# kazuto1011/dusty-gan-v2

Hardware: AMD Instinct MI355X
Metric: range-images/sec (G+D step) on dusty_v2 64x512 (higher is better)
Workload: dtype bf16; 1 GPU; configs[2]: configs/gans/dusty_v2.yaml full G+D train step (G step + D step + lazy R1 + ADA + EMA + Adam), 64x512 synthetic; global_batch=64, per_gpu_batch=64, parallelism=dp1, hip_graph=True, d_epilogue_dtype=fp32, pe_table_precomputed=True

## Files before the change

dusty-gan-v2_amd/csrc/api.hip:

```cpp
#include "common.h"

extern "C" int dgv2_abi_version(void) { return 49; }
```

dusty-gan-v2_amd/dgv2_native/__init__.py:

```python
import ctypes
import os

import torch

_HERE = os.path.dirname(os.path.abspath(__file__))
LIB_PATH = os.environ.get("DGV2_LIB_PATH") or os.path.join(os.path.dirname(_HERE), "lib", "libdgv2.so")

F32, BF16 = 0, 1
ABI_VERSION = 49

_c_int, _c_i64, _c_f32, _c_ptr = ctypes.c_int, ctypes.c_int64, ctypes.c_float, ctypes.c_void_p

SIGNATURES = {
    "dgv2_abi_version": [],
    "dgv2_fused_bias_act": [_c_ptr] * 4 + [_c_i64] * 3 + [_c_int, _c_int, _c_f32, _c_f32, _c_int, _c_ptr],
    "dgv2_bias_grad": [_c_ptr, _c_ptr, _c_i64, _c_i64, _c_i64, _c_int, _c_ptr],
    "dgv2_bias_act_bwd": [_c_ptr] * 4 + [_c_i64, _c_int, _c_f32, _c_f32, _c_ptr, _c_i64, _c_int, _c_ptr],
    "dgv2_bias_act_bwd_rs": [_c_ptr] * 4 + [_c_i64, _c_int, _c_f32, _c_f32, _c_ptr, _c_ptr, _c_i64, _c_int, _c_ptr],
    "dgv2_surface_normal": [_c_ptr, _c_ptr] + [_c_int] * 5 + [_c_ptr],
    "dgv2_mbstd_cat_fwd": [_c_ptr] * 3 + [_c_int] * 7 + [_c_ptr],
    "dgv2_mbstd_cat_bwd": [_c_ptr] * 3 + [_c_int] * 7 + [_c_ptr],
    "dgv2_gemm_x3": [_c_ptr, _c_ptr, _c_i64, _c_ptr, _c_ptr, _c_int, _c_int, _c_i64, _c_int, _c_int, _c_i64, _c_i64, _c_i64,
                     _c_int, _c_f32, _c_ptr],
    "dgv2_pe_wgrad_scratch": [_c_ptr] + [_c_int] * 4,
    "dgv2_pe_wgrad": [_c_ptr, _c_ptr, _c_i64, _c_ptr, _c_ptr] + [_c_int] * 4 + [_c_i64, _c_int, _c_ptr],
    "dgv2_mbstd_cat_fwd_x": [_c_ptr] * 3 + [_c_int] * 8 + [_c_ptr],
    "dgv2_mbstd_cat_bwd_x": [_c_ptr] * 3 + [_c_int] * 8 + [_c_ptr],
    "dgv2_scale_cast": [_c_ptr] * 3 + [_c_i64, _c_int, _c_int, _c_int, _c_ptr],
    "dgv2_upfirdn2d": [_c_ptr] * 3 + [_c_int] * 15 + [_c_ptr],
    "dgv2_resample": [_c_ptr] * 4 + [_c_int] * 19 + [_c_ptr],
    "dgv2_resample_tab": [_c_ptr] * 5 + [_c_int] + [_c_ptr] * 3 + [_c_int] * 10 + [_c_ptr],
    "dgv2_resample_tab_add": [_c_ptr] * 6 + [_c_int] + [_c_ptr] * 3 + [_c_int] * 8 + [_c_ptr],
    "dgv2_resample_tab_add_affine": [_c_ptr] * 8 + [_c_int] + [_c_ptr] * 3 + [_c_int] * 8 + [_c_ptr],
    "dgv2_fourier_feature": [_c_ptr] * 5 + [_c_int] * 8 + [_c_ptr],
    "dgv2_downsample_angle": [_c_ptr] * 4 + [_c_int] * 5 + [_c_ptr],
    "dgv2_bmm_nn": [_c_ptr] * 3 + [_c_int] * 6 + [_c_i64, _c_ptr, _c_int, _c_f32, _c_f32, _c_int, _c_int, _c_ptr],
    "dgv2_bmm_tn": [_c_ptr] * 3 + [_c_int] * 7 + [_c_ptr],
    "dgv2_bmm_nn_cat": [_c_ptr] * 4 + [_c_int] * 5 + [_c_ptr, _c_int, _c_f32, _c_f32, _c_int, _c_int, _c_ptr],
    "dgv2_bmm_nn_cat_sq": [_c_ptr] * 4 + [_c_int] * 5 + [_c_ptr, _c_ptr, _c_int, _c_f32, _c_f32, _c_int, _c_int, _c_ptr, _c_int, _c_ptr,
                           _c_ptr],
    "dgv2_bmm_nn_sq": [_c_ptr] * 3 + [_c_int] * 6 + [_c_i64, _c_ptr, _c_ptr, _c_int, _c_f32, _c_f32, _c_ptr, _c_int, _c_int, _c_ptr, _c_int,
                       _c_ptr, _c_ptr],
    "dgv2_modconv_pe_fwd": [_c_ptr] * 4 + [_c_int] * 5 + [_c_ptr, _c_int, _c_f32, _c_f32, _c_int, _c_ptr],
    "dgv2_modconv_pe_fwd_sq": [_c_ptr] * 4 + [_c_int] * 5 + [_c_ptr, _c_ptr, _c_int, _c_f32, _c_f32, _c_int, _c_ptr, _c_int, _c_ptr,
                               _c_ptr],
    "dgv2_modconv_pe_fwd_head": [_c_ptr] * 4 + [_c_int] * 5 + [_c_ptr, _c_ptr, _c_int, _c_f32, _c_f32, _c_int, _c_ptr, _c_int, _c_ptr,
                                 _c_ptr, _c_ptr, _c_ptr],
    "dgv2_kitti_rows": [_c_ptr, _c_ptr, _c_ptr, _c_int, _c_int, _c_ptr],
    "dgv2_kitti_project": [_c_ptr] * 4 + [_c_int] * 4 + [_c_f32, _c_f32, _c_int, _c_ptr],
    "dgv2_fps_scratch": [_c_ptr, _c_int, _c_int],
    "dgv2_fps": [_c_ptr] * 3 + [_c_int] * 3 + [_c_ptr],
    "dgv2_gather_points": [_c_ptr] * 3 + [_c_int] * 4 + [_c_ptr],
    "dgv2_gather_points_grad": [_c_ptr] * 3 + [_c_int] * 4 + [_c_ptr],
    "dgv2_chamfer_fwd": [_c_ptr] * 6 + [_c_int] * 3 + [_c_ptr],
    "dgv2_nn_search": [_c_ptr] * 4 + [_c_int] * 4 + [_c_ptr],
    "dgv2_chamfer_bwd": [_c_ptr] * 8 + [_c_int] * 3 + [_c_ptr],
    "dgv2_emd_approxmatch": [_c_ptr] * 4 + [_c_int] * 3 + [_c_ptr],
    "dgv2_emd_matchcost": [_c_ptr] * 4 + [_c_int] * 3 + [_c_ptr],
    "dgv2_emd_matchcost_grad": [_c_ptr] * 5 + [_c_int] * 3 + [_c_ptr],
    "dgv2_nsgan_loss": [_c_ptr, _c_ptr, _c_ptr, _c_int, _c_int, _c_f32, _c_ptr, _c_ptr, _c_ptr],
    "dgv2_modconv_pe_dgrad_actbwd": [_c_ptr, _c_ptr, _c_ptr, _c_i64] + [_c_ptr] * 5 + [_c_f32, _c_f32] + [_c_int] * 4 + [_c_ptr],
    "dgv2_colmean_lerp": [_c_ptr, _c_ptr, _c_int, _c_int, _c_i64, _c_f32, _c_ptr],
    "dgv2_d_tail_fwd": [_c_ptr] * 6 + [_c_int, _c_int] + [_c_f32] * 4 + [_c_ptr],
    "dgv2_d_tail_bwd": [_c_ptr] * 7 + [_c_int, _c_int] + [_c_f32] * 4 + [_c_ptr],
    "dgv2_rng_fill": [_c_ptr] * 5 + [_c_int, _c_ptr, _c_ptr],
    "dgv2_modconv_up_fwd": [_c_ptr] * 4 + [_c_int] * 7 + [_c_ptr] * 6 + [_c_int, _c_f32, _c_f32, _c_int, _c_ptr, _c_int, _c_ptr,
                            _c_ptr],
    "dgv2_modconv_up_t_lag": [_c_ptr] * 4 + [_c_f32] + [_c_ptr] * 4 + [_c_int] * 9 + [_c_ptr, _c_int, _c_ptr, _c_ptr],
    "dgv2_fir_same_mfma_q8": [_c_ptr] * 3 + [_c_int] * 4 + [_c_ptr],
    "dgv2_resample_tab_q8": [_c_ptr] * 5 + [_c_int] + [_c_ptr] * 3 + [_c_int] * 7 + [_c_ptr],
    "dgv2_fp8_quant_weights": [_c_ptr] * 6 + [_c_int] + [_c_ptr] * 3,
    "dgv2_fp8_dequant": [_c_ptr, _c_ptr, _c_i64, _c_f32, _c_ptr],
    "dgv2_conv_taps_fp8": [_c_ptr] * 4 + [_c_int] * 14 + [_c_ptr, _c_int, _c_ptr, _c_ptr, _c_int, _c_f32, _c_f32, _c_ptr],
    "dgv2_modconv_up_t": [_c_ptr] * 5 + [_c_f32] + [_c_int] * 9 + [_c_ptr],
    "dgv2_up2_lag_sumsq": [_c_ptr] * 5 + [_c_int] * 5 + [_c_ptr, _c_int, _c_ptr, _c_ptr],
    "dgv2_resample_tab_actbwd": [_c_ptr, _c_ptr, _c_ptr, _c_i64, _c_ptr, _c_ptr, _c_ptr] + [_c_ptr] * 3 + [_c_int] + [_c_ptr] * 3
                                + [_c_int] * 7 + [_c_f32, _c_f32, _c_int, _c_ptr],
    "dgv2_fir_same_mfma_prep": [_c_ptr, _c_i64, _c_ptr] + [_c_ptr] * 3 + [_c_int] + [_c_ptr] * 3 + [_c_int] * 3 + [_c_ptr, _c_ptr],
    "dgv2_fir_same_mfma": [_c_ptr] * 3 + [_c_int] * 4 + [_c_ptr],
    "dgv2_fir_same_mfma_actbwd": [_c_ptr, _c_ptr, _c_ptr, _c_i64, _c_ptr, _c_ptr, _c_ptr, _c_ptr] + [_c_int] * 4
                                 + [_c_f32, _c_f32, _c_ptr],
    "dgv2_resample_tab_sq": [_c_ptr] * 5 + [_c_int] + [_c_ptr] * 3 + [_c_int] * 10 + [_c_ptr, _c_int, _c_ptr, _c_ptr],
    "dgv2_bmm_tn_cat": [_c_ptr] * 4 + [_c_int] * 6 + [_c_ptr],
    "dgv2_lerp_list": [_c_ptr] * 3 + [_c_int, _c_f32, _c_ptr],
    "dgv2_adam_prep": [_c_ptr, _c_ptr, _c_f32, _c_f32, _c_ptr],
    "dgv2_adam_step": [_c_ptr] * 5 + [_c_int, _c_ptr] + [_c_f32] * 4 + [_c_ptr],
    "dgv2_pack2d": [_c_ptr] * 4 + [_c_int] * 3 + [_c_ptr],
    "dgv2_unpack2d": [_c_ptr] * 4 + [_c_int] * 3 + [_c_ptr],
    "dgv2_ema_scalar": [_c_ptr] * 3 + [_c_int] + [_c_f32] * 3 + [_c_int, _c_ptr, _c_int, _c_ptr],
    "dgv2_ema_scalar_group": [_c_ptr, _c_ptr, _c_int, _c_ptr, _c_int] + [_c_f32] * 3 + [_c_int, _c_ptr, _c_ptr],
    "dgv2_bmm_nn_small": [_c_ptr] * 4 + [_c_int] * 5 + [_c_ptr],
    "dgv2_bmm_nn_small_act": [_c_ptr] * 4 + [_c_int] * 4 + [_c_ptr, _c_ptr, _c_f32, _c_f32, _c_ptr, _c_ptr, _c_i64, _c_ptr, _c_int,
                              _c_ptr],
    "dgv2_bmm_tn_small": [_c_ptr] * 3 + [_c_int] * 5 + [_c_ptr],
    "dgv2_head_bwd": [_c_ptr] * 5 + [_c_i64] + [_c_ptr] * 7 + [_c_f32, _c_f32] + [_c_int] * 5 + [_c_ptr],
    "dgv2_transpose_list": [_c_ptr] * 5 + [_c_int] * 3 + [_c_ptr],
    "dgv2_mod_prep_all_fwd": [_c_ptr] * 13 + [_c_ptr, _c_int, _c_int, _c_ptr],
    "dgv2_mod_prep_all_bwd": [_c_ptr, _c_i64] + [_c_ptr] * 15 + [_c_ptr, _c_int, _c_int, _c_ptr, _c_i64, _c_ptr],
    "dgv2_mod_prep_all_bwd_scratch": [_c_ptr, _c_ptr, _c_ptr, _c_int, _c_int],
    "dgv2_mod_prep_fwd": [_c_ptr] * 8 + [_c_int] * 9 + [_c_ptr],
    "dgv2_mod_prep_bwd": [_c_ptr] * 11 + [_c_int] * 9 + [_c_ptr],
    "dgv2_sum_squares": [_c_ptr, _c_ptr, _c_i64, _c_int, _c_int, _c_int, _c_ptr],
    "dgv2_conv_fwd": [_c_ptr] * 3 + [_c_int] * 10 + [_c_ptr, _c_int, _c_f32, _c_f32, _c_int, _c_ptr],
    "dgv2_conv_taps": [_c_ptr] * 3 + [_c_int] * 17 + [_c_ptr] + [_c_int] * 3 + [_c_ptr, _c_ptr, _c_int, _c_f32, _c_f32, _c_int,
                                                                               _c_ptr],
    "dgv2_conv_taps_ex": [_c_ptr] * 3 + [_c_int] * 14 + [_c_ptr, _c_int, _c_int, _c_ptr, _c_int, _c_ptr] + [_c_int] * 3
    + [_c_ptr, _c_ptr, _c_int, _c_f32, _c_f32, _c_int, _c_ptr],
    "dgv2_conv_taps_ld": [_c_ptr, _c_int, _c_ptr, _c_ptr] + [_c_int] * 14 + [_c_ptr, _c_int, _c_int, _c_ptr, _c_int, _c_ptr] + [_c_int] * 3
    + [_c_ptr, _c_ptr, _c_int, _c_f32, _c_f32, _c_int, _c_ptr],
    "dgv2_conv_wgrad_direct": [_c_ptr] * 3 + [_c_int] * 10 + [_c_ptr],
    "dgv2_bmm_tn_stream_scratch": [_c_ptr] + [_c_int] * 6,
    "dgv2_bmm_tn_stream": [_c_ptr, _c_ptr, _c_i64, _c_ptr, _c_ptr] + [_c_int] * 6 + [_c_ptr],
    "dgv2_bmm_tn_stream_x": [_c_ptr, _c_ptr, _c_i64, _c_ptr, _c_ptr] + [_c_int] * 7 + [_c_ptr],
    "dgv2_bmm_tn_stream_ld": [_c_ptr, _c_i64, _c_ptr, _c_i64, _c_ptr, _c_ptr] + [_c_int] * 7 + [_c_ptr],
    "dgv2_conv_weight_bank": [_c_ptr] * 8 + [_c_int, _c_int, _c_ptr],
    "dgv2_conv_weight_bank_ex": [_c_ptr] * 10 + [_c_int, _c_int, _c_ptr],
    "dgv2_glin_fwd": [_c_ptr] * 6 + [_c_int] * 3 + [_c_f32, _c_f32, _c_int, _c_f32, _c_int, _c_ptr, _c_ptr],
    "dgv2_glin_dinput": [_c_ptr, _c_int, _c_ptr, _c_i64, _c_ptr, _c_ptr, _c_ptr, _c_ptr, _c_int, _c_int, _c_int, _c_f32, _c_f32,
                         _c_int, _c_ptr],
    "dgv2_glin_dweight": [_c_ptr] * 7 + [_c_int] * 3 + [_c_f32, _c_f32, _c_f32, _c_ptr, _c_ptr],
    "dgv2_conv3x3_dgrad8": [_c_ptr] * 3 + [_c_int] * 5 + [_c_ptr, _c_int, _c_ptr],
    "dgv2_conv3x3_s2_dgrad8": [_c_ptr] * 3 + [_c_int] * 6 + [_c_ptr],
    "dgv2_conv3x3_x3_wgrad_scratch": [_c_ptr] + [_c_int] * 6,
    "dgv2_conv3x3_x3_wgrad": [_c_ptr, _c_ptr, _c_i64] + [_c_ptr] * 2 + [_c_int] * 7 + [_c_f32, _c_int, _c_ptr, _c_ptr],
    "dgv2_conv_x3_images": [_c_ptr] * 3 + [_c_int] * 2 + [_c_ptr],
    "dgv2_conv3x3_x3_dgrad": [_c_ptr] * 4 + [_c_int] * 6 + [_c_ptr, _c_ptr],
    "dgv2_conv3x3_x3_fwd": [_c_ptr] * 3 + [_c_int] * 6 + [_c_ptr, _c_ptr, _c_int, _c_f32, _c_f32, _c_ptr, _c_ptr],
    "dgv2_conv3x3_fwd8": [_c_ptr] * 3 + [_c_int] * 6 + [_c_ptr, _c_ptr, _c_int, _c_f32, _c_f32, _c_int, _c_ptr],
    "dgv2_conv_wgrad_stream_scratch": [_c_ptr] + [_c_int] * 9,
    "dgv2_conv_wgrad_stream": [_c_ptr, _c_ptr, _c_i64, _c_ptr, _c_ptr] + [_c_int] * 10 + [_c_ptr],
    "dgv2_conv_wgrad_stream_pl": [_c_ptr, _c_ptr, _c_i64, _c_ptr, _c_ptr] + [_c_int] * 9 + [_c_f32, _c_int, _c_int, _c_ptr],
    "dgv2_conv_dgrad": [_c_ptr] * 4 + [_c_int] * 11 + [_c_ptr],
    "dgv2_conv_wgrad": [_c_ptr] * 3 + [_c_int] * 11 + [_c_ptr],
    "dgv2_stem_fwd": [_c_ptr] * 4 + [_c_int] * 5 + [_c_f32, _c_f32, _c_int, _c_ptr],
    "dgv2_stem_bwd_scratch": [_c_ptr] + [_c_int] * 4,
    "dgv2_stem_bwd": [_c_ptr] * 4 + [_c_i64] + [_c_ptr] * 4 + [_c_int] * 5 + [_c_f32, _c_f32, _c_int, _c_ptr],
    "dgv2_stem_bwd_skip": [_c_ptr] * 4 + [_c_i64] + [_c_ptr] * 8 + [_c_int] + [_c_ptr] * 3 + [_c_int] * 8 + [_c_f32, _c_f32, _c_int,
                                                                                                        _c_ptr],
    "dgv2_gen_tail_fwd": [_c_ptr] * 7 + [_c_int] * 3 + [_c_f32] * 3 + [_c_ptr],
    "dgv2_gen_tail_bwd": [_c_ptr] * 11 + [_c_int] * 3 + [_c_f32] * 3 + [_c_ptr],
    "dgv2_ada_apply": [_c_ptr] * 8 + [_c_int] * 5 + [_c_ptr],
    "dgv2_ada_sample": [_c_ptr] * 7 + [_c_int] * 3 + [_c_ptr],
    "dgv2_ada_build": [_c_ptr] * 8 + [_c_int] * 4 + [_c_ptr],
    "dgv2_ada_sample_img": [_c_ptr] * 7 + [_c_int, _c_ptr],
    "dgv2_ada_fold": [_c_ptr] * 11 + [_c_int] * 6 + [_c_ptr],
    "dgv2_ada_apply_img": [_c_ptr] * 11 + [_c_int] * 5 + [_c_ptr],
    "dgv2_coords_convert": [_c_ptr] * 4 + [_c_int] * 3 + [_c_f32] * 3 + [_c_int, _c_ptr],
    "dgv2_msml_prepare": [_c_ptr] * 6 + [_c_int] * 5 + [_c_ptr],
    "dgv2_msml_fwd": [_c_ptr] * 7 + [_c_int] * 7 + [_c_ptr],
    "dgv2_msml_bwd": [_c_ptr] * 9 + [_c_int] * 7 + [_c_ptr],
    "dgv2_coords_convert_bwd": [_c_ptr] * 5 + [_c_int] * 3 + [_c_f32, _c_f32, _c_int, _c_ptr],
    "dgv2_fourier_feature_bwd": [_c_ptr] * 6 + [_c_int] * 8 + [_c_ptr],
}


def _load():
    if not os.path.exists(LIB_PATH):
        raise ImportError(
            f"{LIB_PATH} not found: build it with `make` (or __graft_entry__.build()). "
            "The MI355X path has no CPU fallback."
        )
    lib = ctypes.CDLL(LIB_PATH)
    for name, argtypes in SIGNATURES.items():
        fn = getattr(lib, name)
        fn.argtypes = argtypes
        fn.restype = ctypes.c_int
    got = lib.dgv2_abi_version()
    if got != ABI_VERSION:
        raise ImportError(f"libdgv2.so ABI version {got}, binding expects {ABI_VERSION}")
    return lib


lib = _load()


def dtype_code(t):
    if t.dtype == torch.float32:
        return F32
    if t.dtype == torch.bfloat16:
        return BF16
    raise RuntimeError(f"dgv2: unsupported dtype {t.dtype} (float32 / bfloat16 only)")


def check(*tensors):
    for t in tensors:
        if t is None:
            continue
        if not t.is_cuda:
            raise RuntimeError("dgv2: tensor must be a CUDA/HIP tensor (no CPU fallback)")
        if not t.is_contiguous():
            raise RuntimeError("dgv2: tensor must be contiguous")


# ... 63 lines not shown
```

dusty-gan-v2_amd/gans/models/ops/native/conv.py:

```python
import contextlib
import os
from typing import NamedTuple, Optional

import torch
from torch.autograd import Function

import dgv2_native as N
from . import act_resample as _act_resample
from .act_resample import *
from .modgemm import *


class ConvGeom:
    def __init__(self, kh, kw, stride, pad, ring):
        self.kh, self.kw, self.stride, self.pad, self.ring = kh, kw, stride, pad, int(bool(ring))

    def out_hw(self, H, W):
        return (H + 2 * self.pad - self.kh) // self.stride + 1, (W + 2 * self.pad - self.kw) // self.stride + 1

    @property
    def ring3x3(self):
        return bool(self.ring) and (self.kh, self.kw, self.pad) == (3, 3, 1)


def _kstep(t):
    return 32 if t.dtype == torch.bfloat16 else 16


def _conv_taps(y, x, w3, Hg, Wg, in_stride, ioff, out_stride, ooff, taps, hzero, accumulate=False,
               bias=None, act=0, alpha=0.2, scale=1.0, resid=None):
    B, Hin, Win, Cin = x.shape
    O, wtaps, _ = w3.shape
    _, Hy, Wy, _ = y.shape
    arr = (_ct.c_int * (3 * len(taps)))(*[v for t in taps for v in t])
    N.call("dgv2_conv_taps", N.ptr(y), N.ptr(x), N.ptr(w3), B, Hin, Win, Cin, Hg, Wg, O, Hy, Wy, in_stride,
           ioff[0], ioff[1], out_stride, ooff[0], ooff[1], len(taps), wtaps, arr, int(hzero), 1, int(accumulate),
           N.ptr(bias), N.ptr(resid), act, alpha, scale, _dt(x), N.stream())


_FUSED_DGRAD = os.environ.get("DGV2_NO_FUSED_DGRAD") is None


_S2D8 = os.environ.get("DGV2_NO_S2D8") is None


def _conv_taps_ex(y, x, w3, Hg, Wg, in_stride, ioff, out_stride, classes, taps4, extras, hzero, resid=None, ch0=None):
    B, Hin, Win, Cin = x.shape
    O, wtaps, _ = w3.shape
    _, Hy, Wy, ldy = y.shape
    carr = (_ct.c_int * (2 * len(classes)))(*[v for c in classes for v in c])
    tarr = (_ct.c_int * (4 * len(taps4)))(*[v for t in taps4 for v in t])
    earr = (_ct.c_int * max(5 * len(extras), 1))(*[v for e in extras for v in e])
    if ch0 is not None:
        es = y.element_size()
        rp = None if resid is None else resid.data_ptr() + ch0 * es
        return N.try_call("dgv2_conv_taps_ld", y.data_ptr() + ch0 * es, ldy, N.ptr(x), N.ptr(w3), B, Hin, Win, Cin, Hg, Wg,
                          O, Hy, Wy, in_stride, ioff[0], ioff[1], out_stride, len(classes), carr, len(taps4), wtaps,
                          tarr, len(extras), earr, int(hzero), 1, 0, None, rp, 0, 0.2, 1.0, _dt(x), N.stream())
    return N.try_call("dgv2_conv_taps_ex", N.ptr(y), N.ptr(x), N.ptr(w3), B, Hin, Win, Cin, Hg, Wg, O, Hy, Wy,
                      in_stride, ioff[0], ioff[1], out_stride, len(classes), carr, len(taps4), wtaps, tarr,
                      len(extras), earr, int(hzero), 1, 0, None, N.ptr(resid), 0, 0.2, 1.0, _dt(x), N.stream())


def _direct_ok(g, cin):
    return bool(g.ring) and g.kh == g.kw and (g.kh, g.pad) in ((3, 1), (1, 0)) and g.stride in (1, 2) and cin


_CONV8_IMG = os.environ.get("DGV2_NO_CONV8_IMG") is None


_CONV_X3 = os.environ.get("DGV2_NO_CONV_X3") is None


_X3_AUTO = [False, {}]


@contextlib.contextmanager
def x3_auto(on=True, live=None):
    old = tuple(_X3_AUTO)
    _X3_AUTO[0] = bool(on) and _CONV_X3
    _X3_AUTO[1] = dict(live or {})
    try:
        yield
    finally:
        _X3_AUTO[0], _X3_AUTO[1] = old


def _x3_auto_images(wv, fwd):
    O, kh, kw, Cp = wv.shape
    if (not _X3_AUTO[0] or wv.dtype != torch.float32 or not wv.is_cuda or (kh, kw) != (3, 3) or O % 64 or Cp % 8 or Cp < 64
            or not wv.is_contiguous()):
        return None
    n = 3 * (O // 64) * ((Cp + 31) // 32) if fwd else 3 * (Cp // 64) * (O // 32)
    img = torch.empty(n * 2304 * 8, device=wv.device, dtype=torch.bfloat16)
    N.check(wv)
    N.call("dgv2_conv_x3_images", N.ptr(img) if fwd else None, None if fwd else N.ptr(img), N.ptr(wv), O, Cp, N.stream())
    return img


def _conv_fwd_raw(x, w, g, bias=None, act=0, alpha=0.2, scale=1.0, resid=None, w8=None, xexact=0):
    B, H, W, C = x.shape
    O = w.shape[0]
    Ho, Wo = g.out_hw(H, W)
    N.check(x, w, bias)
    y = torch.empty((B, Ho, Wo, O), device=x.device, dtype=x.dtype)
    if (w8 is not None and _CONV8_IMG and x.dtype == torch.bfloat16 and g.ring3x3 and g.stride in (1, 2)
            and N.try_call("dgv2_conv3x3_fwd8", N.ptr(y), N.ptr(x), N.ptr(w8), B, H, W, C, O, g.stride, N.ptr(bias),
                           N.ptr(resid), act, alpha, scale, _dt(x), N.stream())):
        return y
    if w8 is None and _X3_AUTO[0] and x.dtype == torch.float32 and g.ring3x3 and g.stride == 1 and W % 32 == 0:
        w8 = _x3_auto_images(w, True)
    if (w8 is not None and _CONV_X3 and x.dtype == torch.float32 and w8.dtype == torch.bfloat16 and g.ring3x3 and g.stride == 1
            and N.try_call("dgv2_conv3x3_x3_fwd", N.ptr(y), N.ptr(x), N.ptr(w8), B, H, W, C, min(int(xexact), C), O, N.ptr(bias),
                           N.ptr(resid), act, alpha, scale, N.ptr(N.status_word(x.device)), N.stream())):
        return y
    if _direct_ok(g, C % _kstep(x) == 0):
        taps = [(ky - g.pad, kx - g.pad, ky * g.kw + kx) for ky in range(g.kh) for kx in range(g.kw)]
        _conv_taps(y, x, w.reshape(O, g.kh * g.kw, C), Ho, Wo, g.stride, (0, 0), 1, (0, 0), taps, False,
                   bias=bias, act=act, alpha=alpha, scale=scale, resid=resid)
        return y
    if resid is not None:
        raise RuntimeError("dgv2: fused residual needs the direct conv engine (ring padding, Cin % K-step == 0)")
    N.call("dgv2_conv_fwd", N.ptr(y), N.ptr(x), N.ptr(w), B, H, W, C, O, g.kh, g.kw, g.stride, g.pad, g.ring,
           N.ptr(bias), act, alpha, scale, _dt(x), N.stream())
    return y


def _axis_taps_s2(parity):
    return [(0, 1)] if parity == 0 else [(1, 0), (0, 2)]


def _conv_dgrad8(gy, w8t, xshape, resid):
    B, H, W, C = xshape
    gx = torch.empty(xshape, device=gy.device, dtype=gy.dtype)
    ok = N.try_call("dgv2_conv3x3_dgrad8", N.ptr(gx), N.ptr(gy), N.ptr(w8t), B, H, W, C, gy.shape[3], N.ptr(resid), _dt(gy),
                    N.stream())
    return gx if ok else None


def _conv_dgrad_direct(gy, wt3, g, xshape, resid=None):
    if resid is not None and not (_FUSED_DGRAD and g.kh == 3 and g.stride == 1):
        return _conv_dgrad_direct(gy, wt3, g, xshape) + resid
    B, H, W, C = xshape
    gx = torch.empty(xshape, device=gy.device, dtype=gy.dtype)
    k = g.kh
    if k == 1:
        _conv_taps(gx, gy, wt3, H, W, 1, (0, 0), 1, (0, 0), [(0, 0, 0)], True)
        return gx
    if g.stride == 1:
        taps = [(1 - ky, 1 - kx, ky * 3 + kx) for ky in range(3) for kx in range(3)]
        extras = [(0, 1 - kx, kx, 0, 0) for kx in range(3)] + [(0, 1 - kx, 6 + kx, 0, H - 1) for kx in range(3)]
        tail = C % 64
        if _FUSED_DGRAD and C > 128 and tail in (16, 32) and B * H * W <= 32768:
            main = C - tail
            t4 = [t + (0,) for t in taps]
            if (_conv_taps_ex(gx, gy, wt3[:main], H, W, 1, (0, 0), 1, [(0, 0)], t4, extras, True, resid=resid, ch0=0)
                    and _conv_taps_ex(gx, gy, wt3[main:], H, W, 1, (0, 0), 1, [(0, 0)], t4, extras, True, resid=resid,
                                      ch0=main)):
                return gx
        if _FUSED_DGRAD and _conv_taps_ex(gx, gy, wt3, H, W, 1, (0, 0), 1, [(0, 0)], [t + (0,) for t in taps], extras,
                                          True, resid=resid):
            return gx
        if resid is not None:
            return _conv_dgrad_direct(gy, wt3, g, xshape) + resid
        _conv_taps(gx, gy, wt3, H, W, 1, (0, 0), 1, (0, 0), taps, True)
        _conv_taps(gx, gy, wt3, 1, W, 1, (0, 0), 1, (0, 0), [(0, 1 - kx, kx) for kx in range(3)], True, True)
        _conv_taps(gx, gy, wt3, 1, W, 1, (H - 1, 0), 1, (H - 1, 0), [(0, 1 - kx, 6 + kx) for kx in range(3)], True,
                   True)
        return gx
    if _S2D8 and gy.dtype == torch.bfloat16 and g.ring and C % 128 == 0 and wt3.is_contiguous():
        if N.try_call("dgv2_conv3x3_s2_dgrad8", N.ptr(gx), N.ptr(gy), N.ptr(wt3), B, H // 2, W // 2, C, gy.shape[3], _dt(gy),
                      N.stream()):
            return gx
    classes, taps4, extras = [], [], []
    for ph in (0, 1):
        for pw in (0, 1):
            c = len(classes)
            classes.append((ph, pw))
            taps4 += [(dy, dx, ky * 3 + kx, c) for dy, ky in _axis_taps_s2(ph) for dx, kx in _axis_taps_s2(pw)]
            if ph == 0:
                extras += [(0, dx, kx, c, 0) for dx, kx in _axis_taps_s2(pw)]
    if _FUSED_DGRAD and _conv_taps_ex(gx, gy, wt3, H // 2, W // 2, 1, (0, 0), 2, classes, taps4, extras, True):
        return gx
    for ph in (0, 1):
        for pw in (0, 1):
            taps = [(dy, dx, ky * 3 + kx) for dy, ky in _axis_taps_s2(ph) for dx, kx in _axis_taps_s2(pw)]
            _conv_taps(gx, gy, wt3, H // 2, W // 2, 1, (0, 0), 2, (ph, pw), taps, True)
    for pw in (0, 1):
        taps = [(0, dx, kx) for dx, kx in _axis_taps_s2(pw)]
        _conv_taps(gx, gy, wt3, 1, W // 2, 1, (0, 0), 2, (0, pw), taps, True, True)
    return gx


def _conv_dgrad_raw(gy, w, g, xshape, wt=None, resid=None, w8t=None):
    B, H, W, C = xshape
    O = gy.shape[3]
    if (w8t is not None and _CONV8_IMG and gy.dtype == torch.bfloat16 and g.ring3x3 and g.stride == 1
            and w8t.dtype == gy.dtype):
        N.check(gy, w8t, resid)
        gx = _conv_dgrad8(gy, w8t, xshape, resid)
        if gx is not None:
            return gx
    if (w8t is not None and _CONV_X3 and gy.dtype == torch.float32 and w8t.dtype == torch.bfloat16 and wt is not None
            and g.ring3x3 and g.stride == 1 and getattr(w8t, "_dgv2_clive", None)):
        clive = w8t._dgv2_clive
        N.check(gy, w8t, wt, resid)
        gx = torch.empty(xshape, device=gy.device, dtype=gy.dtype)
        if N.try_call("dgv2_conv3x3_x3_dgrad", N.ptr(gx), N.ptr(gy), N.ptr(w8t), N.ptr(wt), B, H, W, int(clive), C, O,
                      N.ptr(resid), N.stream()):
            return gx
    if wt is None:
        c = getattr(w, "_dgv2_vals_t", None)
        if c is not None and c[0] == w._version:
            wt = c[1]
        else:
            wt = w.permute(3, 1, 2, 0).contiguous()
            w._dgv2_vals_t = (w._version, wt)
    N.check(gy, wt, resid)
    if (w is not None and _X3_AUTO[0] and gy.dtype == torch.float32 and g.ring3x3 and g.stride == 1
            and W % 32 == 0 and H >= 2 and C % 64 <= 16):
        w3t = _x3_auto_images(w, False)
        if w3t is not None:
            gx = torch.empty(xshape, device=gy.device, dtype=gy.dtype)
            if N.try_call("dgv2_conv3x3_x3_dgrad", N.ptr(gx), N.ptr(gy), N.ptr(w3t), N.ptr(wt), B, H, W,
                          int(_X3_AUTO[1].get(C, C)), C, O, N.ptr(resid), N.stream()):
                return gx
    even = g.stride == 1 or (H % 2 == 0 and W % 2 == 0)
    if _direct_ok(g, O % _kstep(gy) == 0) and even and not (g.kh == 1 and g.stride == 2):
        return _conv_dgrad_direct(gy, wt.reshape(C, g.kh * g.kw, O), g, xshape, resid)
    if resid is not None:
        return _conv_dgrad_raw(gy, w, g, xshape, wt) + resid
    gx = torch.empty(xshape, device=gy.device, dtype=gy.dtype)
    scratch = None
    if g.pad > 0:
        scratch = torch.empty((B, H + 2 * g.pad, W + 2 * g.pad, C), device=gy.device, dtype=gy.dtype)
    N.call("dgv2_conv_dgrad", N.ptr(gx), N.ptr(scratch), N.ptr(gy), N.ptr(wt), B, H, W, C, O, g.kh, g.kw, g.stride,
           g.pad, g.ring, _dt(gy), N.stream())
    return gx


_WGRAD_DIRECT_MAXC = int(os.environ.get("DGV2_WGRAD_DIRECT_MAXC", "64"))


_WGRAD_STREAM = os.environ.get("DGV2_NO_WGRAD_STREAM") is None


_WGRAD_SCRATCH = {}


_TN_STREAM = os.environ.get("DGV2_NO_TN_STREAM") is None


_TN_SCRATCH = {}


_LIB_WGRAD = os.environ.get("DGV2_NO_LIB_WGRAD") is None


def _bmm_tn_small(gy, x, B, P, I, O, batch_sum=False):
    lanes = 256 // max(I * x.element_size() // 16, 1)
    ns = 1
    while B * ns < 1024 and P % (2 * ns) == 0 and P // (2 * ns) >= lanes * 16:
        ns *= 2
    parts = torch.empty((B, ns, O, I), device=x.device, dtype=torch.float32)
    if not N.try_call("dgv2_bmm_tn_small", N.ptr(parts), N.ptr(gy), N.ptr(x), B * ns, P // ns, I, O, _dt(x), N.stream()):
        return None
    if batch_sum:
        return parts.sum(dim=(0, 1))
    return parts.view(B, O, I) if ns == 1 else parts.sum(dim=1)


def _conv_wgrad_raw(gy, x, g, gscale=None, x3=None, xexact=0, out=None):
    B, H, W, C = x.shape
    O = gy.shape[3]
    N.check(gy, x)
    if x3 is None and _X3_AUTO[0]:
        x3 = int(_X3_AUTO[1].get(C, C))
    if (x3 and _CONV_X3 and x.dtype == torch.float32 and g.ring3x3 and g.stride == 1
            and O % 128 == 0 and C >= 64 and C % 8 == 0 and W % 32 == 0 and 0 <= x3 - C // 64 * 64 <= 16):
        key = ("x3", B, H, W, C, int(x3), O)
        if key not in _WGRAD_SCRATCH:
            n = _ct.c_int64(0)
            N.call("dgv2_conv3x3_x3_wgrad_scratch", _ct.addressof(n), B, H, W, C, int(x3), O)
            _WGRAD_SCRATCH[key] = n.value
        scratch = torch.empty(_WGRAD_SCRATCH[key], device=x.device, dtype=torch.float32)
        gw3 = (out if (out is not None and gscale is not None and tuple(out.shape) == (O, C, 3, 3)) else
               torch.empty((O, C, 3, 3) if gscale is not None else (O, 3, 3, C), device=x.device, dtype=torch.float32))
        if N.try_call("dgv2_conv3x3_x3_wgrad", N.ptr(gw3), N.ptr(scratch), scratch.numel(), N.ptr(gy), N.ptr(x), B, H, W, C,
                      int(x3), min(int(xexact), C), O, 1.0 if gscale is None else float(gscale), int(gscale is not None),
                      N.ptr(N.status_word(x.device)), N.stream()):
            return gw3 if gscale is None else gw3.permute(0, 2, 3, 1)
    stream_ok = (_WGRAD_STREAM and g.kh == g.kw and (g.kh, g.pad) in ((3, 1), (1, 0)) and g.stride in (1, 2)
                 and C % (16 // x.element_size()) == 0 and O % (16 // x.element_size()) == 0)
    if gscale is not None:
        if not stream_ok:
            gp = _conv_wgrad_raw(gy, x, g).permute(0, 3, 1, 2)
            return torch.mul(gp, gscale, out=torch.empty(gp.shape, device=x.device)).permute(0, 2, 3, 1)
        gw = (out if (out is not None and tuple(out.shape) == (O, C, g.kh, g.kw)) else
              torch.empty((O, C, g.kh, g.kw), device=x.device, dtype=torch.float32))
    else:
        gw = torch.empty((O, g.kh, g.kw, C), device=x.device, dtype=torch.float32)
    if stream_ok:
        key = (B, H, W, C, O, g.kh, g.stride, g.pad, _dt(x))
        if key not in _WGRAD_SCRATCH:
            n = _ct.c_int64(0)
            N.call("dgv2_conv_wgrad_stream_scratch", _ct.addressof(n), B, H, W, C, O, g.kh, g.stride, g.pad, _dt(x))
            _WGRAD_SCRATCH[key] = n.value
        scratch = torch.empty(_WGRAD_SCRATCH[key], device=x.device, dtype=torch.float32)
        N.call("dgv2_conv_wgrad_stream_pl", N.ptr(gw), N.ptr(scratch), scratch.numel(), N.ptr(gy), N.ptr(x), B, H, W,
# ... 625 lines not shown
```

include/dgv2.h:

```cpp
#ifndef DGV2_H
#define DGV2_H

#include <stdint.h>

#ifdef __cplusplus
extern "C" {
#endif

#define DGV2_F32 0
#define DGV2_BF16 1
#define DGV2_FP8 2
#define DGV2_EINVAL (-1)
#define DGV2_ENOTSUP (-3)

#define DGV2_STATUS_X_INEXACT 1
#define DGV2_STATUS_FIR_TABLE 2

int dgv2_abi_version(void);

int dgv2_fused_bias_act(void* y, const void* x, const void* bias, const void* ref,
                        int64_t size_x, int64_t step_b, int64_t size_b,
                        int act, int grad, float alpha, float scale, int dtype, void* stream);

int dgv2_bias_grad(float* gb, const void* x, int64_t size_x, int64_t step_b, int64_t size_b,
// ... 156 lines not shown
int dgv2_mbstd_cat_bwd(void* gx, const void* gout, const void* x, int B, int P, int C, int Cp, int splits,
                       int group, int dtype, void* stream);
int dgv2_gemm_x3(float* c, float* scratch, int64_t scratch_elems, const float* a, const float* b, int I, int J,
                 int64_t T, int a_trans, int b_trans, int64_t lda, int64_t ldb, int64_t ldo, int splits, float scale,
                 void* stream);
int dgv2_pe_wgrad_scratch(int64_t* elems, int B, int P, int O, int Ks);
int dgv2_pe_wgrad(float* gw, float* scratch, int64_t scratch_elems, const void* g, const void* pe, int B, int P, int O,
                  int Ks, int64_t ldo, int col0, void* stream);
int dgv2_mbstd_cat_fwd_x(void* out, float* scratch, const void* x, int B, int P, int C, int Cp, int splits, int group,
                         int xdtype, int ydtype, void* stream);
int dgv2_mbstd_cat_bwd_x(void* gx, const void* gout, const void* x, int B, int P, int C, int Cp, int splits, int group,
                         int xdtype, int gdtype, void* stream);

int dgv2_conv_fwd(void* y, const void* x, const void* w, int B, int H, int W, int C, int O,
                  int kh, int kw, int stride, int pad, int ring,
                  const float* bias, int act, float alpha, float scale, int dtype, void* stream);
int dgv2_conv_dgrad(void* gx, void* gxp_scratch, const void* gy, const void* wt,
                    int B, int H, int W, int C, int O,
                    int kh, int kw, int stride, int pad, int ring, int dtype, void* stream);
int dgv2_conv_wgrad(float* gw, const void* gy, const void* x, int B, int H, int W, int C, int O,
                    int kh, int kw, int stride, int pad, int ring, int dtype, void* stream);

int dgv2_conv_wgrad_direct(float* gw, const void* gy, const void* x, int B, int H, int W, int C, int O,
                           int k, int stride, int pad, int ring, int dtype, void* stream);

int dgv2_bmm_tn_stream_scratch(int64_t* elems, int B, int H, int W, int C, int O, int dtype);
int dgv2_bmm_tn_stream(float* gw, float* scratch, int64_t scratch_elems, const void* gy, const void* x,
                       int B, int H, int W, int C, int O, int dtype, void* stream);
int dgv2_bmm_tn_stream_x(float* gw, float* scratch, int64_t scratch_elems, const void* gy, const void* x,
                         int x_shared, int B, int H, int W, int C, int O, int dtype, void* stream);
int dgv2_bmm_tn_stream_ld(float* gw, int64_t ldo, float* scratch, int64_t scratch_elems, const void* gy, const void* x,
                          int x_shared, int B, int H, int W, int C, int O, int dtype, void* stream);

int dgv2_conv_weight_bank(void* const* wf, void* const* wt, const float* const* src, const int* O,
                          const int* C, const int* Cpad, const int* kk, const float* scale, int L,
                          int dtype, void* stream);
int dgv2_conv_weight_bank_ex(void* const* wf, void* const* wt, void* const* w8, void* const* w8t,
                             const float* const* src, const int* O, const int* C, const int* Cpad, const int* kk,
                             const float* scale, int L, int dtype, void* stream);
int dgv2_conv3x3_fwd8(void* y, const void* x, const void* w8, int B, int Hin, int Win, int Cin, int O, int stride,
                      const float* bias, const void* resid, int act, float alpha, float scale, int dtype, void* stream);
int dgv2_conv3x3_dgrad8(void* gx, const void* gy, const void* w8t, int B, int H, int W, int C, int O, const void* resid,
                        int dtype, void* stream);
int dgv2_conv3x3_s2_dgrad8(void* gx, const void* gy, const void* wt, int B, int Hg, int Wg, int C, int O, int dtype,
                           void* stream);

int dgv2_conv3x3_x3_fwd(void* y, const void* x, const void* w3, int B, int H, int W, int Cx, int x_exact, int O,
                        const float* bias, const void* resid, int act, float alpha, float scale, int* status,
                        void* stream);
int dgv2_conv3x3_x3_dgrad(void* gx, const void* gy, const void* w3t, const void* wt, int B, int H, int W, int C, int ldx,
                          int O, const void* resid, void* stream);
int dgv2_conv3x3_x3_wgrad(float* gw, float* scratch, int64_t scratch_elems, const void* gy, const void* x, int B, int H,
                          int W, int C, int clive, int x_exact, int O, float scale, int param_layout, int* status,
                          void* stream);
int dgv2_conv3x3_x3_wgrad_scratch(int64_t* elems, int B, int H, int W, int C, int clive, int O);
int dgv2_conv_x3_images(void* w3, void* w3t, const void* w, int O, int Cp, void* stream);

int dgv2_conv_wgrad_stream_scratch(int64_t* elems, int B, int H, int W, int C, int O, int k, int stride,
                                   int pad, int dtype);
int dgv2_conv_wgrad_stream(float* gw, float* scratch, int64_t scratch_elems, const void* gy, const void* x,
                           int B, int H, int W, int C, int O, int k, int stride, int pad, int ring,
                           int dtype, void* stream);
int dgv2_conv_wgrad_stream_pl(float* gw, float* scratch, int64_t scratch_elems, const void* gy, const void* x,
                              int B, int H, int W, int C, int O, int k, int stride, int pad, int ring,
                              float scale, int param_layout, int dtype, void* stream);

int dgv2_conv_taps(void* y, const void* x, const void* w, int B, int Hin, int Win, int Cin,
                   int Hg, int Wg, int O, int Hy, int Wy, int in_stride, int ioff_h, int ioff_w,
                   int out_stride, int ooff_h, int ooff_w, int ntaps, int wtaps, const int* taps_host,
                   int hzero, int ring, int accumulate, const float* bias, const void* resid, int act,
                   float alpha, float scale, int dtype, void* stream);
int dgv2_conv_taps_ex(void* y, const void* x, const void* w, int B, int Hin, int Win, int Cin, int Hg,
                      int Wg, int O, int Hy, int Wy, int in_stride, int ioff_h, int ioff_w,
                      int out_stride, int ncls, const int* cls_host, int ntaps, int wtaps,
                      const int* taps_host, int nextra, const int* extras_host, int hzero, int ring,
                      int accumulate, const float* bias, const void* resid, int act, float alpha,
                      float scale, int dtype, void* stream);
int dgv2_conv_taps_ld(void* y, int ldy, const void* x, const void* w, int B, int Hin, int Win, int Cin, int Hg,
                      int Wg, int O, int Hy, int Wy, int in_stride, int ioff_h, int ioff_w, int out_stride, int ncls,
                      const int* cls_host, int ntaps, int wtaps, const int* taps_host, int nextra,
                      const int* extras_host, int hzero, int ring, int accumulate, const float* bias,
                      const void* resid, int act, float alpha, float scale, int dtype, void* stream);

int dgv2_stem_fwd(void* y, const float* x, const float* w, const float* bias, int B, int H, int W, int O,
                  int ring, float alpha, float scale, int ydtype, void* stream);
int dgv2_stem_bwd_scratch(int64_t* elems, int B, int H, int W, int O);
int dgv2_stem_bwd(float* gx, float* gw, float* gb, float* scratch, int64_t scratch_elems, const void* gy,
                  const void* y, const float* x, const float* w, int B, int H, int W, int O, int ring,
                  float alpha, float scale, int dtype, void* stream);
int dgv2_stem_bwd_skip(float* gx, float* gw, float* gb, float* scratch, int64_t scratch_elems, const void* gy, const void* y,
                       const float* x, const float* w, const void* gsk, const int* idx_h, const float* coef_h,
                       const int* cnt_h, int Eh, const int* idx_w, const float* coef_w, const int* cnt_w, int Ew, int Hs,
                       int Ws, int B, int H, int W, int O, int ring, float alpha, float scale, int dtype, void* stream);

int dgv2_gen_tail_fwd(float* image, float* image_orig, float* logit, float* mask,
                      const float* skip, const float* shift, const float* u,
                      int B, int H, int W, float out_scale, float raydrop_const, float temperature,
                      void* stream);
int dgv2_gen_tail_bwd(float* g_skip, float* scratch, const float* g_image, const float* g_image_orig,
                      const float* g_logit, const float* g_mask,
                      const float* image_orig, const float* logit, const float* mask, const float* u,
                      const float* shift, int B, int H, int W, float out_scale, float raydrop_const,
                      float temperature, void* stream);

int dgv2_ada_apply(float* y, const float* x, const float* Ay, const float* kx, const int* off,
                   const int* sgn, const float* a, const float* c, int B, int H, int W, int K,
                   int transpose, void* stream);

int dgv2_ada_sample(float* gaff, float* a, float* c, const float* u, const float* n, const float* p,
                    const float* policy_host, int B, int H, int W, void* stream);
int dgv2_ada_build(float* Ay, float* kx, int* off, int* sgn, const float* gaff, const float* M1y,
                   const float* M1x, const float* taps, int B, int H, int W, int K, void* stream);

int dgv2_ada_sample_img(float* g, float* sigma, float* cut, const float* u2, const float* n2, const float* p,
                        const float* policy_host, int B, void* stream);
int dgv2_ada_fold(float* Ay2, float* kx2, int* off2, float* c2, const float* Ay, const float* kx, const int* off,
                  const int* sgn, const float* c, const float* g, const float* fbank, int B, int H, int W, int K,
                  int NB, int T, void* stream);
int dgv2_ada_apply_img(float* y, const float* x, const float* Ay, const float* kx, const int* off, const int* sgn,
                       const float* a, const float* c, const float* cut, const float* sigma, const float* eps, int B,
                       int H, int W, int K, int transpose, void* stream);

int dgv2_coords_convert(float* out, const float* in, const float* mask, const float* angle,
                        int B, int H, int W, float min_depth, float max_depth, float raydrop_const,
                        int mode, void* stream);

int dgv2_surface_normal(float* out, const float* points, int B, int H, int W, int d, int mode, void* stream);

int dgv2_nsgan_loss(float* stats, float* gy, const float* y, int n_real, int n_fake, float gy_scale, float* sign_cum,
                    float* n_cum, void* stream);

int dgv2_d_tail_fwd(float* y, float* a, const float* h, const float* b1, const float* w2, const float* b2, int B, int K,
                    float alpha, float act_scale, float scale2, float gain2, void* stream);
int dgv2_d_tail_bwd(float* gh, float* gb1, float* gw2, float* gb2, const float* gy, const float* a, const float* w2,
                    int B, int K, float alpha, float act_scale, float scale2, float gain2, void* stream);

int dgv2_colmean_lerp(float* dst, const float* src, int B, int K, int64_t ld, float w, void* stream);

int dgv2_rng_fill(float* const* out, const int64_t* count, const int* kind, const float* a, const float* b, int nseg,
                  uint64_t* state, void* stream);

int dgv2_kitti_rows(int* row, int* counts, const float* pts, int n, int H, void* stream);
int dgv2_kitti_project(float* out, unsigned long long* key, const float* pts, const int* row, int n, int H, int W,
                       int Wout, float min_depth, float max_depth, int apply_mask, void* stream);

int dgv2_fps_scratch(int64_t* floats, int B, int n);
int dgv2_fps(int* idxs, float* temp, const float* xyz, int B, int n, int m, void* stream);
int dgv2_gather_points(float* out, const float* points, const int* idx, int B, int C, int n, int m, void* stream);
int dgv2_gather_points_grad(float* grad_points, const float* grad_out, const int* idx, int B, int C, int n, int m,
                            void* stream);

int dgv2_chamfer_fwd(float* dist1, int* idx1, float* dist2, int* idx2, const float* xyz1, const float* xyz2, int B,
                     int n, int m, void* stream);
int dgv2_nn_search(float* dist, int* idx, const float* xyz, const float* ref, int B, int n, int m, int ref_shared,
                   void* stream);
int dgv2_chamfer_bwd(float* gxyz1, float* gxyz2, const float* xyz1, const float* xyz2, const float* gdist1,
                     const float* gdist2, const int* idx1, const int* idx2, int B, int n, int m, void* stream);

int dgv2_emd_approxmatch(float* match, float* temp, const float* xyz1, const float* xyz2, int B, int n, int m,
                         void* stream);
int dgv2_emd_matchcost(float* cost, const float* match, const float* xyz1, const float* xyz2, int B, int n, int m,
                       void* stream);
int dgv2_emd_matchcost_grad(float* grad1, float* grad2, const float* match, const float* xyz1, const float* xyz2, int B,
                            int n, int m, void* stream);

int dgv2_fir_same_mfma_q8(void* y8, const void* x, const void* bands, int B, int C, int H, int W, void* stream);
// ... 39 lines not shown
```

Measured before the change: 5432 range-images/s.

## Add dedicated MFMA kernel for bf16 1x1 convolution forward and dgrad

Introduces a specialized 1x1 convolution kernel that stages a weight slab in LDS and streams pixel tiles through bf16 MFMA 16x16x32, with an optional fused residual add and non-temporal stores. The Python conv paths route stride-1, pad-0 1x1 convs without bias or activation (forward) and 1x1 dgrad to this kernel ahead of the generic direct/tap paths. The aim is to cut overhead of the general tap-based conv for pointwise layers such as skip or projection convs. It only applies for bf16 with K up to 512 and K, M multiples of 32; other shapes fall back.

```diff
diff --git a/dusty-gan-v2_amd/csrc/api.hip b/dusty-gan-v2_amd/csrc/api.hip
--- a/dusty-gan-v2_amd/csrc/api.hip
+++ b/dusty-gan-v2_amd/csrc/api.hip
@@ -1,3 +1,3 @@
 #include "common.h"
 
-extern "C" int dgv2_abi_version(void) { return 49; }
+extern "C" int dgv2_abi_version(void) { return 50; }
diff --git a/dusty-gan-v2_amd/csrc/conv1x1.hip b/dusty-gan-v2_amd/csrc/conv1x1.hip
--- /dev/null
+++ b/dusty-gan-v2_amd/csrc/conv1x1.hip
@@ -0,0 +1,186 @@
+#include "common.h"
+
+namespace {
+
+constexpr int kPixTile = 32;
+constexpr int kWaves = 4;
+constexpr int kMaxK = 512;
+
+struct C1Params {
+  bf16_t* out;
+  const bf16_t* in;
+  const bf16_t* w;
+  const bf16_t* resid;
+  int64_t N;
+  int K, M;
+  int nt;
+};
+
+template <int MF, int KC>
+__global__ __launch_bounds__(256, 4) void conv1x1_kernel(const C1Params p) {
+  extern __shared__ uint4 s_w[];
+  const int K = p.K, M = p.M;
+  const int kslots = K >> 3, rs = kslots + 1;
+  const int m0 = blockIdx.y * (16 * MF);
+  const int wslots = 16 * MF * kslots;
+  for (int i0 = threadIdx.x; i0 < wslots; i0 += 4 * 256) {
+    uint4 v[4];
+#pragma unroll
+    for (int u = 0; u < 4; ++u) {
+      const int i = min(i0 + u * 256, wslots - 1);
+      v[u] = *reinterpret_cast<const uint4*>(p.w + (int64_t)m0 * K + (int64_t)i * 8);
+    }
+#pragma unroll
+    for (int u = 0; u < 4; ++u) {
+      const int i = min(i0 + u * 256, wslots - 1);
+      s_w[(i / kslots) * rs + i % kslots] = v[u];
+    }
+  }
+  __syncthreads();
+
+  const int lane = threadIdx.x & 63, wave = threadIdx.x >> 6;
+  const int lr = lane & 15, lc = lane >> 4;
+  const int co = (lc & 1) ? 16 + 4 * (lc - 1) : 4 * lc;
+  const int64_t ntiles = (p.N + kPixTile - 1) / kPixTile;
+  const int ksteps = K >> 5;
+
+  for (int64_t t = (int64_t)blockIdx.x * kWaves + wave; t < ntiles; t += (int64_t)gridDim.x * kWaves) {
+    int64_t pix[2];
+    const bf16_t* ip[2];
+#pragma unroll
+    for (int nf = 0; nf < 2; ++nf) {
+      pix[nf] = t * kPixTile + nf * 16 + lr;
+      const int64_t pc = pix[nf] < p.N ? pix[nf] : p.N - 1;
+      ip[nf] = p.in + pc * K + lc * 8;
+    }
+    uint4 rr[2][MF / 2];
+    if (p.resid) {
+#pragma unroll
+      for (int nf = 0; nf < 2; ++nf) {
+        const int64_t pc = pix[nf] < p.N ? pix[nf] : p.N - 1;
+#pragma unroll
+        for (int mp = 0; mp < MF / 2; ++mp)
+          rr[nf][mp] = *reinterpret_cast<const uint4*>(p.resid + pc * M + m0 + mp * 32 + co);
+      }
+    }
+    f32x4 acc[MF][2];
+#pragma unroll
+    for (int mf = 0; mf < MF; ++mf)
+#pragma unroll
+      for (int nf = 0; nf < 2; ++nf) acc[mf][nf] = f32x4{0.f, 0.f, 0.f, 0.f};
+
+    for (int k0 = 0; k0 < ksteps; k0 += KC) {
+      bf16x8 b[KC][2];
+#pragma unroll
+      for (int kc = 0; kc < KC; ++kc)
+#pragma unroll
+        for (int nf = 0; nf < 2; ++nf) b[kc][nf] = *reinterpret_cast<const bf16x8*>(ip[nf] + (k0 + kc) * 32);
+#pragma unroll
+      for (int kc = 0; kc < KC; ++kc) {
+#pragma unroll
+        for (int mf = 0; mf < MF; ++mf) {
+          union { uint4 u; bf16x8 v; } a;
+          a.u = s_w[(mf * 16 + lr) * rs + (k0 + kc) * 4 + lc];
+#pragma unroll
+          for (int nf = 0; nf < 2; ++nf)
+            acc[mf][nf] = __builtin_amdgcn_mfma_f32_16x16x32_bf16(a.v, b[kc][nf], acc[mf][nf], 0, 0, 0);
+        }
+      }
+    }
+
+#pragma unroll
+    for (int nf = 0; nf < 2; ++nf) {
+#pragma unroll
+      for (int mp = 0; mp < MF / 2; ++mp) {
+        float fa[4], fb[4];
+#pragma unroll
+        for (int r = 0; r < 4; ++r) {
+          fa[r] = acc[2 * mp][nf][r];
+          fb[r] = acc[2 * mp + 1][nf][r];
+        }
+        vec16<bf16_t> v;
+        pack_pair_bf16(fa, fb, lc, v.raw);
+        if (p.resid) {
+          vec16<bf16_t> r;
+          r.raw = rr[nf][mp];
+#pragma unroll
+          for (int j = 0; j < 8; ++j) v.set(j, v.get(j) + r.get(j));
+        }
+        if (pix[nf] < p.N) {
+          bf16_t* q = p.out + pix[nf] * M + m0 + mp * 32 + co;
+          if (p.nt) v.store_nt(q); else v.store(q);
+        }
+      }
+    }
+  }
+}
+
+int device_cus() {
+  static int cus = 0;
+  if (cus == 0) {
+    int dev = 0, n = 0;
+    if (hipGetDevice(&dev) != hipSuccess || hipDeviceGetAttribute(&n, hipDeviceAttributeMultiprocessorCount, dev) != hipSuccess
+        || n <= 0)
+      n = 256;
+    cus = n;
+  }
+  return cus;
+}
+
+template <int MF, int KC>
+int launch(const C1Params& p, hipStream_t st) {
+  const size_t lds = (size_t)16 * MF * (p.K / 8 + 1) * 16;
+  static bool attr = false;
+  if (!attr) {
+    if (hipFuncSetAttribute(reinterpret_cast<const void*>(&conv1x1_kernel<MF, KC>), hipFuncAttributeMaxDynamicSharedMemorySize,
+                            16 * MF * (kMaxK / 8 + 1) * 16) != hipSuccess)
+      return DGV2_EINVAL;
+    attr = true;
+  }
+  const int slabs = p.M / (16 * MF);
+  const int64_t want = (p.N + kPixTile * kWaves - 1) / (kPixTile * kWaves);
+  int per_cu = (int)((160 * 1024) / (lds + 512));
+  per_cu = per_cu > 4 ? 4 : per_cu;
+  int64_t gx = ((int64_t)device_cus() * per_cu + slabs - 1) / slabs;
+  gx = gx < want ? gx : want;
+  conv1x1_kernel<MF, KC><<<dim3((unsigned)gx, (unsigned)slabs), 256, lds, st>>>(p);
+  DGV2_RETURN_LAST();
+}
+
+int conv1x1_run(void* out, const void* in, const void* w, const void* resid, int64_t N, int K, int M, int dtype,
+                hipStream_t st) {
+  if (!out || !in || !w || N <= 0 || K <= 0 || M <= 0) return DGV2_EINVAL;
+  if (dtype != DGV2_BF16 || K % 32 || M % 32 || K > kMaxK || !aligned16(out) || !aligned16(in) || !aligned16(w)
+      || (resid && !aligned16(resid)))
+    return DGV2_ENOTSUP;
+  C1Params p;
+  p.out = reinterpret_cast<bf16_t*>(out);
+  p.in = reinterpret_cast<const bf16_t*>(in);
+  p.w = reinterpret_cast<const bf16_t*>(w);
+  p.resid = reinterpret_cast<const bf16_t*>(resid);
+  p.N = N; p.K = K; p.M = M;
+  p.nt = (!resid && nt_output(N * M * (int64_t)sizeof(bf16_t))) ? 1 : 0;
+  const int kc = K % 128 == 0 ? 4 : K % 64 == 0 ? 2 : 1;
+  if (M % 64 == 0) {
+    if (kc == 4) return launch<4, 4>(p, st);
+    if (kc == 2) return launch<4, 2>(p, st);
+    return launch<4, 1>(p, st);
+  }
+  if (kc == 4) return launch<2, 4>(p, st);
+  if (kc == 2) return launch<2, 2>(p, st);
+  return launch<2, 1>(p, st);
+}
+
+}
+
+extern "C" int dgv2_conv1x1_fwd(void* y, const void* x, const void* wf, int B, int P, int C, int O, const void* resid,
+                                int dtype, void* stream) {
+  if (B <= 0 || P <= 0) return DGV2_EINVAL;
+  return conv1x1_run(y, x, wf, resid, (int64_t)B * P, C, O, dtype, reinterpret_cast<hipStream_t>(stream));
+}
+
+extern "C" int dgv2_conv1x1_dgrad(void* gx, const void* gy, const void* wt, int B, int P, int C, int O, const void* resid,
+                                  int dtype, void* stream) {
+  if (B <= 0 || P <= 0) return DGV2_EINVAL;
+  return conv1x1_run(gx, gy, wt, resid, (int64_t)B * P, O, C, dtype, reinterpret_cast<hipStream_t>(stream));
+}
diff --git a/dusty-gan-v2_amd/dgv2_native/__init__.py b/dusty-gan-v2_amd/dgv2_native/__init__.py
--- a/dusty-gan-v2_amd/dgv2_native/__init__.py
+++ b/dusty-gan-v2_amd/dgv2_native/__init__.py
@@ -7,7 +7,7 @@
 LIB_PATH = os.environ.get("DGV2_LIB_PATH") or os.path.join(os.path.dirname(_HERE), "lib", "libdgv2.so")
 
 F32, BF16 = 0, 1
-ABI_VERSION = 49
+ABI_VERSION = 50
 
 _c_int, _c_i64, _c_f32, _c_ptr = ctypes.c_int, ctypes.c_int64, ctypes.c_float, ctypes.c_void_p
 
@@ -109,6 +109,8 @@
     "dgv2_conv_taps_ld": [_c_ptr, _c_int, _c_ptr, _c_ptr] + [_c_int] * 14 + [_c_ptr, _c_int, _c_int, _c_ptr, _c_int, _c_ptr] + [_c_int] * 3
     + [_c_ptr, _c_ptr, _c_int, _c_f32, _c_f32, _c_int, _c_ptr],
     "dgv2_conv_wgrad_direct": [_c_ptr] * 3 + [_c_int] * 10 + [_c_ptr],
+    "dgv2_conv1x1_fwd": [_c_ptr] * 3 + [_c_int] * 4 + [_c_ptr, _c_int, _c_ptr],
+    "dgv2_conv1x1_dgrad": [_c_ptr] * 3 + [_c_int] * 4 + [_c_ptr, _c_int, _c_ptr],
     "dgv2_bmm_tn_stream_scratch": [_c_ptr] + [_c_int] * 6,
     "dgv2_bmm_tn_stream": [_c_ptr, _c_ptr, _c_i64, _c_ptr, _c_ptr] + [_c_int] * 6 + [_c_ptr],
     "dgv2_bmm_tn_stream_x": [_c_ptr, _c_ptr, _c_i64, _c_ptr, _c_ptr] + [_c_int] * 7 + [_c_ptr],
diff --git a/dusty-gan-v2_amd/gans/models/ops/native/conv.py b/dusty-gan-v2_amd/gans/models/ops/native/conv.py
--- a/dusty-gan-v2_amd/gans/models/ops/native/conv.py
+++ b/dusty-gan-v2_amd/gans/models/ops/native/conv.py
@@ -98,6 +98,21 @@
     return img
 
 
+_CONV1X1 = os.environ.get("DGV2_NO_CONV1X1") is None
+
+
+def _conv1x1(entry, out, a, w, B, P, C, O, resid):
+    if not _CONV1X1 or a.dtype != torch.bfloat16 or w.dtype != a.dtype or not w.is_contiguous():
+        return False
+    if resid is not None and (resid.dtype != a.dtype or not resid.is_contiguous()):
+        return False
+    return N.try_call(entry, N.ptr(out), N.ptr(a), N.ptr(w), B, P, C, O, N.ptr(resid), _dt(a), N.stream())
+
+
+def _is_1x1(g):
+    return (g.kh, g.kw, g.stride, g.pad) == (1, 1, 1, 0)
+
+
 def _conv_fwd_raw(x, w, g, bias=None, act=0, alpha=0.2, scale=1.0, resid=None, w8=None, xexact=0):
     B, H, W, C = x.shape
     O = w.shape[0]
@@ -113,6 +128,8 @@
     if (w8 is not None and _CONV_X3 and x.dtype == torch.float32 and w8.dtype == torch.bfloat16 and g.ring3x3 and g.stride == 1
             and N.try_call("dgv2_conv3x3_x3_fwd", N.ptr(y), N.ptr(x), N.ptr(w8), B, H, W, C, min(int(xexact), C), O, N.ptr(bias),
                            N.ptr(resid), act, alpha, scale, N.ptr(N.status_word(x.device)), N.stream())):
+        return y
+    if _is_1x1(g) and bias is None and act == 0 and _conv1x1("dgv2_conv1x1_fwd", y, x, w, B, H * W, C, O, resid):
         return y
     if _direct_ok(g, C % _kstep(x) == 0):
         taps = [(ky - g.pad, kx - g.pad, ky * g.kw + kx) for ky in range(g.kh) for kx in range(g.kw)]
@@ -225,6 +242,10 @@
             if N.try_call("dgv2_conv3x3_x3_dgrad", N.ptr(gx), N.ptr(gy), N.ptr(w3t), N.ptr(wt), B, H, W,
                           int(_X3_AUTO[1].get(C, C)), C, O, N.ptr(resid), N.stream()):
                 return gx
+    if _is_1x1(g) and gy.is_contiguous():
+        gx = torch.empty(xshape, device=gy.device, dtype=gy.dtype)
+        if _conv1x1("dgv2_conv1x1_dgrad", gx, gy, wt, B, H * W, C, O, resid):
+            return gx
     even = g.stride == 1 or (H % 2 == 0 and W % 2 == 0)
     if _direct_ok(g, O % _kstep(gy) == 0) and even and not (g.kh == 1 and g.stride == 2):
         return _conv_dgrad_direct(gy, wt.reshape(C, g.kh * g.kw, O), g, xshape, resid)
diff --git a/include/dgv2.h b/include/dgv2.h
--- a/include/dgv2.h
+++ b/include/dgv2.h
@@ -262,6 +262,11 @@
                       const int* extras_host, int hzero, int ring, int accumulate, const float* bias,
                       const void* resid, int act, float alpha, float scale, int dtype, void* stream);
 
+int dgv2_conv1x1_fwd(void* y, const void* x, const void* wf, int B, int P, int C, int O, const void* resid, int dtype,
+                     void* stream);
+int dgv2_conv1x1_dgrad(void* gx, const void* gy, const void* wt, int B, int P, int C, int O, const void* resid,
+                       int dtype, void* stream);
+
 int dgv2_stem_fwd(void* y, const float* x, const float* w, const float* bias, int B, int H, int W, int O,
                   int ring, float alpha, float scale, int ydtype, void* stream);
 int dgv2_stem_bwd_scratch(int64_t* elems, int B, int H, int W, int O);
```

After: 5555 range-images/s (median of 6 runs). +2.3%, better.
